# NVlabs/EmerNeRF

Hardware: NVIDIA H100
Metric: training rays/sec (8192-ray batch) (higher is better)
Workload: dtype f32

## Files before the change

### emernerf_b200/csrc/field_wgrad.cu

```cuda
#include "common.cuh"
#include "tc_common.cuh"

namespace emer {
namespace fw {

using namespace emer::tc;

constexpr int TR = 16;
constexpr int STAGES = 3;
constexpr int THREADS = 384;
constexpr int PROD_REGS = 56, CONS_REGS = 224;
constexpr int MIN_TILES = 4;

constexpr int BAR_FULL = 1, BAR_EMPTY = 3, BAR_RING = 5, BAR_PROD = 5 + STAGES;

constexpr int PANEL64 = TR * 64 * 4, PANEL8 = TR * 8 * 4;
constexpr int P_DZB = 0, P_DF = 2 * PANEL64, P_DSEM = 4 * PANEL64, P_DZ0 = 6 * PANEL64, P_DZ1 = 8 * PANEL64,
              P_DZ2 = 10 * PANEL64, P_BYTES = P_DZ2 + 2 * PANEL8;

template <int KE, bool HEAD>
struct Stage {
    static constexpr int LD_ENC = KE + 4, LD64 = 68, LD128 = 132, LD_D1 = HEAD ? LD128 : LD64;
    static constexpr int ENC = 0, HB = ENC + TR * LD_ENC, DZB = HB + TR * LD64, DSEM = DZB + TR * LD64,
                         D1 = DSEM + TR * LD64, DF = D1 + (HEAD ? 64 : 0), HG = D1 + TR * LD_D1, H1 = HG + TR * LD128,
                         DZ1 = H1 + TR * LD64, DZ2 = DZ1 + TR * LD64;
    static constexpr int FLOATS = HEAD ? DZ2 + TR * 3 : HG;
};

struct Params {
    const float* enc; int64_t ld_enc;
    const float *hb, *hg, *h1, *dz2, *dz1, *d1, *dzb, *d_sem;
    float *dwb0, *dbb0, *dwb1, *dbb1;
    float *dw0g, *dw1h, *dw1g; int64_t ld_w0, ld_w1;
    float *dw2, *db2;
    int64_t n;
};

__device__ __forceinline__ void cp_async16(float* dst, const float* src, int bytes) {
    asm volatile("cp.async.cg.shared.global [%0], [%1], 16, %2;\n" ::"r"(smem_u32(dst)), "l"(src), "r"(bytes) : "memory");
}
__device__ __forceinline__ void cp_async_commit() { asm volatile("cp.async.commit_group;\n" ::: "memory"); }
template <int N>
__device__ __forceinline__ void cp_async_wait() { asm volatile("cp.async.wait_group %0;\n" ::"n"(N) : "memory"); }
__device__ __forceinline__ void bar_sync(int id, int count) { asm volatile("bar.sync %0, %1;\n" ::"r"(id), "r"(count) : "memory"); }
__device__ __forceinline__ void bar_arrive(int id, int count) { asm volatile("bar.arrive %0, %1;\n" ::"r"(id), "r"(count) : "memory"); }

template <int W>
__device__ __forceinline__ void copy_rows(float* dst, const float* src, int64_t ld, int64_t row0, int rows_left, int t) {
    constexpr int CPR = W / 4, CHUNKS = TR * CPR;
    const float* s = src + row0 * ld;
#pragma unroll
    for (int k = 0; k < (CHUNKS + 127) / 128; ++k) {
        const int c = t + 128 * k;
        if (CHUNKS % 128 == 0 || c < CHUNKS) {
            const int r = c / CPR, j = c % CPR;
            const bool ok = r < rows_left;
            cp_async16(dst + r * (W + 4) + 4 * j, ok ? s + r * ld + 4 * j : src, ok ? 16 : 0);
        }
    }
}

template <int B, int KE, bool HEAD>
__device__ __forceinline__ void split_col(const float* st, uint8_t* pan, int col, bool sem, float& dbs) {
    using S = Stage<KE, HEAD>;
    constexpr int soff = B == 0 ? S::DZB : B == 1 ? S::DF : B == 2 ? S::DSEM : B == 3 ? S::D1 : B == 4 ? S::DZ1 : S::DZ2;
    constexpr int sld = B == 1 || B == 3 ? S::LD_D1 : (B == 5 ? 3 : S::LD64);
    constexpr int rows = B == 5 ? 8 : 64;
    constexpr int pb = B == 0 ? P_DZB : B == 1 ? P_DF : B == 2 ? P_DSEM : B == 3 ? P_DZ0 : B == 4 ? P_DZ1 : P_DZ2;
    if constexpr (B >= 3 && !HEAD) return;
    if ((B == 2 && !sem) || (B == 5 && col >= 8)) return;
    const bool real = B != 5 || col < 3;
    const float* z = st + soff + (real ? col : 0);
#pragma unroll
    for (int ks = 0; ks < 2; ++ks) {
#pragma unroll
        for (int h = 0; h < 2; ++h) {
            float v[4], hi[4], lo[4];
#pragma unroll
            for (int j = 0; j < 4; ++j) {
                v[j] = real ? z[(8 * ks + 2 * j + h) * sld] : 0.0f;
                split(v[j], hi[j], lo[j]);
                dbs += v[j];
            }
            uint8_t* dst = pan + pb + (2 * ks + h) * rows * 16 + col * 16;
            *reinterpret_cast<float4*>(dst) = make_float4(hi[0], hi[1], hi[2], hi[3]);
            *reinterpret_cast<float4*>(dst + TR * rows * 4) = make_float4(lo[0], lo[1], lo[2], lo[3]);
        }
    }
}

template <int FV>
__device__ __forceinline__ void load_a(const float* x, int ld, int f0, int q, uint32_t (&hi)[2][4], uint32_t (&lo)[2][4]) {
    const int f1 = f0 + 8;
#pragma unroll
    for (int ks = 0; ks < 2; ++ks) {
        const float* ra = x + (8 * ks + 2 * q) * ld;
        const float* rb = ra + ld;
        frag_split(f0 < FV ? ra[f0] : 0.0f, f0 < FV ? rb[f0] : 0.0f, f1 < FV ? ra[f1] : 0.0f, f1 < FV ? rb[f1] : 0.0f,
                   hi[ks], lo[ks]);
    }
}

template <int N>
__device__ __forceinline__ void mma_tile(float (&acc)[N / 2], const uint32_t (&hi)[2][4], const uint32_t (&lo)[2][4],
                                         uint32_t panel) {
#pragma unroll
    for (int ks = 0; ks < 2; ++ks)
        mma3<N>(acc, hi[ks], lo[ks], b_desc(panel, N, ks, 0), b_desc(panel + TR * N * 4, N, ks, 0), 1);
}

template <int N>
__device__ __forceinline__ void flush(const float (&acc)[N / 2], float* dw, int64_t ld, int fv, int ov, int f0, int q) {
#pragma unroll
    for (int j = 0; j < N / 8; ++j) {
#pragma unroll
        for (int e = 0; e < 4; ++e) {
            const int f = e < 2 ? f0 : f0 + 8, o = 8 * j + 2 * q + (e & 1);
            if (f < fv && o < ov) atomicAdd(dw + (int64_t)o * ld + f, acc[4 * j + e]);
        }
    }
}

template <int KE, bool HEAD>
__global__ void __launch_bounds__(THREADS, 1) field_wgrad_kernel(const __grid_constant__ Params p) {
    using S = Stage<KE, HEAD>;
    extern __shared__ __align__(128) uint8_t smem[];
    float* ring = reinterpret_cast<float*>(smem + 2 * P_BYTES);
    const int tid = threadIdx.x, lane = tid & 31, q = lane & 3;
    const int wgi = __shfl_sync(0xffffffffu, tid >> 7, 0);
    const bool sem = p.d_sem != nullptr;
    const int64_t n_tiles = (p.n + TR - 1) / TR;
    const int64_t my_tiles = (n_tiles - blockIdx.x + gridDim.x - 1) / gridDim.x;

    if (wgi == 0) {
        asm volatile("setmaxnreg.dec.sync.aligned.u32 %0;\n" ::"n"(PROD_REGS));
        auto issue = [&](int64_t i, int slot) {
            if (i < my_tiles) {
                const int64_t row0 = (blockIdx.x + i * gridDim.x) * TR;
                const int rows_left = p.n - row0 < TR ? (int)(p.n - row0) : TR;
                float* st = ring + slot * S::FLOATS;
                copy_rows<KE>(st + S::ENC, p.enc, p.ld_enc, row0, rows_left, tid);
                copy_rows<64>(st + S::HB, p.hb, 64, row0, rows_left, tid);
                copy_rows<64>(st + S::DZB, p.dzb, 64, row0, rows_left, tid);
                if (sem) copy_rows<64>(st + S::DSEM, p.d_sem, 64, row0, rows_left, tid);
                copy_rows<HEAD ? 128 : 64>(st + S::D1, p.d1 + (HEAD ? 0 : 64), 128, row0, rows_left, tid);
                if constexpr (HEAD) {
                    copy_rows<128>(st + S::HG, p.hg, 128, row0, rows_left, tid);
                    copy_rows<64>(st + S::H1, p.h1, 64, row0, rows_left, tid);
                    copy_rows<64>(st + S::DZ1, p.dz1, 64, row0, rows_left, tid);
                    if (tid < TR * 3 / 4) {
                        const int left = rows_left * 12 - 16 * tid;
                        const int b = left <= 0 ? 0 : (left < 16 ? left : 16);
                        cp_async16(st + S::DZ2 + 4 * tid, b ? p.dz2 + row0 * 3 + 4 * tid : p.dz2, b);
                    }
                }
            }
            cp_async_commit();
        };
        const int col = tid & 63, half = __shfl_sync(0xffffffffu, tid >> 6, 0);
        float db0 = 0.0f, db1 = 0.0f, db2 = 0.0f;
        issue(0, 0);
        issue(1, 1);
        int slot = 0;
        for (int64_t i = 0; i < my_tiles; ++i, slot = slot + 1 == STAGES ? 0 : slot + 1) {
            const int pb = (int)(i & 1), prev = slot == 0 ? STAGES - 1 : slot - 1;
            if (i >= 1 && i + 2 < my_tiles) bar_sync(BAR_RING + prev, THREADS);
            issue(i + 2, prev);
            if (i >= 2) bar_sync(BAR_EMPTY + pb, THREADS);
            cp_async_wait<2>();
            bar_sync(BAR_PROD, 128);
            const float* st = ring + slot * S::FLOATS;
            uint8_t* pan = smem + pb * P_BYTES;
            if (half == 0) {
                split_col<0, KE, HEAD>(st, pan, col, sem, db0);
                split_col<2, KE, HEAD>(st, pan, col, sem, db1);
                split_col<4, KE, HEAD>(st, pan, col, sem, db2);
            } else {
                split_col<1, KE, HEAD>(st, pan, col, sem, db0);
                split_col<3, KE, HEAD>(st, pan, col, sem, db1);
                split_col<5, KE, HEAD>(st, pan, col, sem, db2);
            }
            fence_async_proxy();
            bar_arrive(BAR_FULL + pb, THREADS);
        }
        cp_async_wait<0>();
        if (half == 0) {
            atomicAdd(p.dbb0 + col, db0);
            if (sem) atomicAdd(p.dbb1 + 64 + col, db1);
        } else {
            atomicAdd(p.dbb1 + col, db0);
            if (HEAD && col < 3) atomicAdd(p.db2 + col, db2);
        }
    } else {
        asm volatile("setmaxnreg.inc.sync.aligned.u32 %0;\n" ::"n"(CONS_REGS));
        const uint32_t pan0 = smem_u32(smem);
        const int f0 = 16 * ((tid >> 5) & 3) + (lane >> 2);
        float a0[32], a1[32], a2[32], a3[4];
#pragma unroll
        for (int i = 0; i < 32; ++i) a0[i] = a1[i] = a2[i] = 0.0f;
#pragma unroll
        for (int i = 0; i < 4; ++i) a3[i] = 0.0f;

        int slot = 0;
        for (int64_t i = 0; i < my_tiles; ++i, slot = slot + 1 == STAGES ? 0 : slot + 1) {
            const int pb = (int)(i & 1);
            bar_sync(BAR_FULL + pb, THREADS);
            const float* st = ring + slot * S::FLOATS;
            const uint32_t pan = pan0 + (uint32_t)pb * P_BYTES;
            uint32_t h0[2][4], l0[2][4], h1[2][4], l1[2][4], h2[2][4], l2[2][4];
            if (wgi == 1) {
                load_a<KE>(st + S::ENC, S::LD_ENC, f0, q, h0, l0);
                if (HEAD) load_a<64>(st + S::HG + 64, S::LD128, f0, q, h1, l1);
            } else {
                load_a<64>(st + S::HB, S::LD64, f0, q, h0, l0);
                if (HEAD) {
                    load_a<64>(st + S::HG, S::LD128, f0, q, h1, l1);
                    load_a<64>(st + S::H1, S::LD64, f0, q, h2, l2);
                }
            }
            if (i + STAGES < my_tiles) bar_arrive(BAR_RING + slot, THREADS);
            wg_fence();
            if (wgi == 1) {
                mma_tile<64>(a0, h0, l0, pan + P_DZB);
                if (HEAD) {
                    mma_tile<64>(a1, h1, l1, pan + P_DZ0);
                    mma_tile<64>(a2, h1, l1, pan + P_DZ1);
                }
            } else {
                mma_tile<64>(a0, h0, l0, pan + P_DF);
                if (sem) mma_tile<64>(a2, h0, l0, pan + P_DSEM);
                if (HEAD) {
                    mma_tile<64>(a1, h1, l1, pan + P_DZ1);
                    mma_tile<8>(a3, h2, l2, pan + P_DZ2);
                }
            }
            wg_commit();
            wg_wait0();
            if (i + 2 < my_tiles) bar_arrive(BAR_EMPTY + pb, THREADS);
        }

        if (wgi == 1) {
            flush<64>(a0, p.dwb0, KE, KE, 64, f0, q);
            if (HEAD) {
                flush<64>(a1, p.dw0g, p.ld_w0, 64, 64, f0, q);
                flush<64>(a2, p.dw1g, p.ld_w1, 64, 64, f0, q);
            }
        } else {
            flush<64>(a0, p.dwb1, 64, 64, 64, f0, q);
            if (sem) flush<64>(a2, p.dwb1 + 64 * 64, 64, 64, 64, f0, q);
            if (HEAD) {
                flush<64>(a1, p.dw1h, p.ld_w1, 64, 64, f0, q);
                flush<8>(a3, p.dw2, 64, 64, 3, f0, q);
            }
        }
    }
}

template <int KE, bool HEAD>
static int launch_t(const Params& p, cudaStream_t st) {
    constexpr int smem = 2 * P_BYTES + STAGES * Stage<KE, HEAD>::FLOATS * 4;
    static_assert(smem <= 227 * 1024, "field_wgrad_kernel: shared memory");
    static bool configured[64] = {false};
    const int dev = current_device();
    if (!configured[dev]) {
        cudaError_t e = cudaFuncSetAttribute(field_wgrad_kernel<KE, HEAD>, cudaFuncAttributeMaxDynamicSharedMemorySize, smem);
        if (e != cudaSuccess) {
            set_error("emer_field_wgrad: cudaFuncSetAttribute(%d): %s", smem, cudaGetErrorString(e));
            return -2;
        }
        configured[dev] = true;
    }
    int64_t grid = sm_count();
    const int64_t ctas = ceil_div(ceil_div(p.n, TR), MIN_TILES);
    if (grid > ctas) grid = ctas;
    field_wgrad_kernel<KE, HEAD><<<(unsigned)grid, THREADS, smem, st>>>(p);
    return check_launch("emer_field_wgrad");
}

template <bool HEAD>
static int launch_h(const Params& p, int k_enc, cudaStream_t st) {
    if (k_enc == 32) return launch_t<32, HEAD>(p, st);
    if (k_enc == 40) return launch_t<40, HEAD>(p, st);
    return launch_t<64, HEAD>(p, st);
}

}
}

extern "C" int emer_field_wgrad(const float* enc, int64_t ld_enc, int k_enc, const float* hb, const float* hg,
                                const float* h1, const float* dz2, const float* dz1, const float* d1, const float* dzb,
                                const float* d_sem, int n_feat, float* dwb0, float* dbb0, float* dwb1, float* dbb1,
                                float* dw0g, int64_t ld_w0, float* dw1h, float* dw1g, int64_t ld_w1, float* dw2,
                                float* db2, int64_t n, void* stream) {
    if (n == 0) return 0;
    EMER_REQUIRE(enc && hb && d1 && dzb && dwb0 && dbb0 && dwb1 && dbb1, "emer_field_wgrad: NULL pointer");
    EMER_REQUIRE(!dz2 || (hg && h1 && dz1 && dw0g && dw1h && dw1g && dw2 && db2),
                 "emer_field_wgrad: NULL pointer among the colour head's buffers");
    EMER_REQUIRE(k_enc == 32 || k_enc == 40 || k_enc == 64, "emer_field_wgrad: k_enc=%d must be 32, 40 or 64", k_enc);
    EMER_REQUIRE(n_feat == 64 || n_feat == 128, "emer_field_wgrad: n_feat=%d must be 64 or 128", n_feat);
    EMER_REQUIRE(!d_sem || n_feat == 128, "emer_field_wgrad: d_sem needs n_feat = 128");
    EMER_REQUIRE(ld_enc % 4 == 0 && ld_enc >= k_enc, "emer_field_wgrad: ld_enc=%lld (need a multiple of 4, >= k_enc)",
                 (long long)ld_enc);
    EMER_REQUIRE(!dz2 || (ld_w0 >= 64 && ld_w1 >= 64), "emer_field_wgrad: ld_w0=%lld ld_w1=%lld shorter than a block",
                 (long long)ld_w0, (long long)ld_w1);
    EMER_REQUIRE((((uintptr_t)enc | (uintptr_t)hb | (uintptr_t)hg | (uintptr_t)h1 | (uintptr_t)dz2 | (uintptr_t)dz1 |
                   (uintptr_t)d1 | (uintptr_t)dzb | (uintptr_t)d_sem) & 15) == 0,
                 "emer_field_wgrad: row buffers must be 16-byte aligned");
    emer::fw::Params p{enc, ld_enc, hb, hg, h1, dz2, dz1, d1, dzb, d_sem, dwb0, dbb0, dwb1, dbb1,
                       dw0g, dw1h, dw1g, ld_w0, ld_w1, dw2, db2, n};
    const cudaStream_t st = (cudaStream_t)stream;
    return dz2 ? emer::fw::launch_h<true>(p, k_enc, st) : emer::fw::launch_h<false>(p, k_enc, st);
}
```

Measured before the change: 2.287 million.

## Load weight-gradient row tiles with TMA and mbarriers, double-buffer consumer fragments

Replaces the per-thread cp.async row copies in the producer warpgroup with TMA bulk tensor copies issued by a single thread and tracked by per-slot mbarriers with expected transaction bytes. Consumers now also wait on the mbarrier. The consumer loop is restructured to load the next tile's A fragments while the current wgmma runs. This aims to cut producer instruction overhead and overlap fragment loads with the MMAs, at the cost of host-side tensor-map encoding on every launch, more consumer registers, and an int32 row limit.

```diff
diff --git a/emernerf_b200/csrc/field_wgrad.cu b/emernerf_b200/csrc/field_wgrad.cu
--- a/emernerf_b200/csrc/field_wgrad.cu
+++ b/emernerf_b200/csrc/field_wgrad.cu
@@ -1,3 +1,6 @@
+#include <cuda.h>
+#include <cudaTypedefs.h>
+
 #include "common.cuh"
 #include "tc_common.cuh"
 
@@ -12,7 +15,7 @@
 constexpr int PROD_REGS = 56, CONS_REGS = 224;
 constexpr int MIN_TILES = 4;
 
-constexpr int BAR_FULL = 1, BAR_EMPTY = 3, BAR_RING = 5, BAR_PROD = 5 + STAGES;
+constexpr int BAR_FULL = 1, BAR_EMPTY = 3, BAR_RING = 5, RING_COUNT = 256 + 32;
 
 constexpr int PANEL64 = TR * 64 * 4, PANEL8 = TR * 8 * 4;
 constexpr int P_DZB = 0, P_DF = 2 * PANEL64, P_DSEM = 4 * PANEL64, P_DZ0 = 6 * PANEL64, P_DZ1 = 8 * PANEL64,
@@ -24,40 +27,42 @@
     static constexpr int ENC = 0, HB = ENC + TR * LD_ENC, DZB = HB + TR * LD64, DSEM = DZB + TR * LD64,
                          D1 = DSEM + TR * LD64, DF = D1 + (HEAD ? 64 : 0), HG = D1 + TR * LD_D1, H1 = HG + TR * LD128,
                          DZ1 = H1 + TR * LD64, DZ2 = DZ1 + TR * LD64;
-    static constexpr int FLOATS = HEAD ? DZ2 + TR * 3 : HG;
+    static constexpr int FLOATS = HEAD ? DZ2 + 64 : HG;
+    static constexpr int TX_BYTES = 4 * TR * (LD_ENC + 2 * LD64 + LD_D1 + (HEAD ? LD128 + 2 * LD64 : 0)) + (HEAD ? 4 * TR * 3 : 0);
+    static constexpr int TX_SEM = 4 * TR * LD64;
 };
 
 struct Params {
-    const float* enc; int64_t ld_enc;
-    const float *hb, *hg, *h1, *dz2, *dz1, *d1, *dzb, *d_sem;
+    CUtensorMap enc, hb, dzb, d_sem, d1, hg, h1, dz1, dz2;
+    bool sem;
     float *dwb0, *dbb0, *dwb1, *dbb1;
     float *dw0g, *dw1h, *dw1g; int64_t ld_w0, ld_w1;
     float *dw2, *db2;
     int64_t n;
 };
 
-__device__ __forceinline__ void cp_async16(float* dst, const float* src, int bytes) {
-    asm volatile("cp.async.cg.shared.global [%0], [%1], 16, %2;\n" ::"r"(smem_u32(dst)), "l"(src), "r"(bytes) : "memory");
-}
-__device__ __forceinline__ void cp_async_commit() { asm volatile("cp.async.commit_group;\n" ::: "memory"); }
-template <int N>
-__device__ __forceinline__ void cp_async_wait() { asm volatile("cp.async.wait_group %0;\n" ::"n"(N) : "memory"); }
 __device__ __forceinline__ void bar_sync(int id, int count) { asm volatile("bar.sync %0, %1;\n" ::"r"(id), "r"(count) : "memory"); }
 __device__ __forceinline__ void bar_arrive(int id, int count) { asm volatile("bar.arrive %0, %1;\n" ::"r"(id), "r"(count) : "memory"); }
 
-template <int W>
-__device__ __forceinline__ void copy_rows(float* dst, const float* src, int64_t ld, int64_t row0, int rows_left, int t) {
-    constexpr int CPR = W / 4, CHUNKS = TR * CPR;
-    const float* s = src + row0 * ld;
-#pragma unroll
-    for (int k = 0; k < (CHUNKS + 127) / 128; ++k) {
-        const int c = t + 128 * k;
-        if (CHUNKS % 128 == 0 || c < CHUNKS) {
-            const int r = c / CPR, j = c % CPR;
-            const bool ok = r < rows_left;
-            cp_async16(dst + r * (W + 4) + 4 * j, ok ? s + r * ld + 4 * j : src, ok ? 16 : 0);
-        }
-    }
+__device__ __forceinline__ void mbar_init(uint32_t bar, int count) {
+    asm volatile("mbarrier.init.shared::cta.b64 [%0], %1;\n" ::"r"(bar), "r"(count) : "memory");
+}
+__device__ __forceinline__ void mbar_arrive_tx(uint32_t bar, int bytes) {
+    asm volatile("mbarrier.arrive.expect_tx.shared::cta.b64 _, [%0], %1;\n" ::"r"(bar), "r"(bytes) : "memory");
+}
+__device__ __forceinline__ void mbar_wait(uint32_t bar, uint32_t parity) {
+    asm volatile(
+        "{\n.reg .pred p;\nWAIT:\n"
+        "mbarrier.try_wait.parity.shared::cta.b64 p, [%0], %1;\n"
+        "@!p bra WAIT;\n}\n" ::"r"(bar), "r"(parity) : "memory");
+}
+__device__ __forceinline__ void copy_box(float* dst, const CUtensorMap& m, int row0, uint32_t bar) {
+    asm volatile("cp.async.bulk.tensor.2d.shared::cluster.global.mbarrier::complete_tx::bytes [%0], [%1, {%2, %3}], [%4];\n"
+                 ::"r"(smem_u32(dst)), "l"(&m), "r"(0), "r"(row0), "r"(bar) : "memory");
+}
+__device__ __forceinline__ void copy_box_1d(float* dst, const CUtensorMap& m, int x0, uint32_t bar) {
+    asm volatile("cp.async.bulk.tensor.1d.shared::cluster.global.mbarrier::complete_tx::bytes [%0], [%1, {%2}], [%3];\n"
+                 ::"r"(smem_u32(dst)), "l"(&m), "r"(x0), "r"(bar) : "memory");
 }
 
 template <int B, int KE, bool HEAD>
@@ -126,49 +131,55 @@
     using S = Stage<KE, HEAD>;
     extern __shared__ __align__(128) uint8_t smem[];
     float* ring = reinterpret_cast<float*>(smem + 2 * P_BYTES);
+    const uint32_t landed = smem_u32(ring + STAGES * S::FLOATS);
     const int tid = threadIdx.x, lane = tid & 31, q = lane & 3;
     const int wgi = __shfl_sync(0xffffffffu, tid >> 7, 0);
-    const bool sem = p.d_sem != nullptr;
+    const bool sem = p.sem;
     const int64_t n_tiles = (p.n + TR - 1) / TR;
     const int64_t my_tiles = (n_tiles - blockIdx.x + gridDim.x - 1) / gridDim.x;
+
+    if (tid < STAGES) mbar_init(landed + 8 * tid, 1);
+    asm volatile("fence.mbarrier_init.release.cluster;\n" ::: "memory");
+    __syncthreads();
 
     if (wgi == 0) {
         asm volatile("setmaxnreg.dec.sync.aligned.u32 %0;\n" ::"n"(PROD_REGS));
         auto issue = [&](int64_t i, int slot) {
-            if (i < my_tiles) {
-                const int64_t row0 = (blockIdx.x + i * gridDim.x) * TR;
-                const int rows_left = p.n - row0 < TR ? (int)(p.n - row0) : TR;
-                float* st = ring + slot * S::FLOATS;
-                copy_rows<KE>(st + S::ENC, p.enc, p.ld_enc, row0, rows_left, tid);
-                copy_rows<64>(st + S::HB, p.hb, 64, row0, rows_left, tid);
-                copy_rows<64>(st + S::DZB, p.dzb, 64, row0, rows_left, tid);
-                if (sem) copy_rows<64>(st + S::DSEM, p.d_sem, 64, row0, rows_left, tid);
-                copy_rows<HEAD ? 128 : 64>(st + S::D1, p.d1 + (HEAD ? 0 : 64), 128, row0, rows_left, tid);
-                if constexpr (HEAD) {
-                    copy_rows<128>(st + S::HG, p.hg, 128, row0, rows_left, tid);
-                    copy_rows<64>(st + S::H1, p.h1, 64, row0, rows_left, tid);
-                    copy_rows<64>(st + S::DZ1, p.dz1, 64, row0, rows_left, tid);
-                    if (tid < TR * 3 / 4) {
-                        const int left = rows_left * 12 - 16 * tid;
-                        const int b = left <= 0 ? 0 : (left < 16 ? left : 16);
-                        cp_async16(st + S::DZ2 + 4 * tid, b ? p.dz2 + row0 * 3 + 4 * tid : p.dz2, b);
-                    }
-                }
-            }
-            cp_async_commit();
+            const int row0 = (int)((blockIdx.x + i * gridDim.x) * TR);
+            const uint32_t bar = landed + 8 * slot;
+            float* st = ring + slot * S::FLOATS;
+            fence_async_proxy();
+            mbar_arrive_tx(bar, S::TX_BYTES + (sem ? S::TX_SEM : 0));
+            copy_box(st + S::ENC, p.enc, row0, bar);
+            copy_box(st + S::HB, p.hb, row0, bar);
+            copy_box(st + S::DZB, p.dzb, row0, bar);
+            if (sem) copy_box(st + S::DSEM, p.d_sem, row0, bar);
+            copy_box(st + S::D1, p.d1, row0, bar);
+            if constexpr (HEAD) {
+                copy_box(st + S::HG, p.hg, row0, bar);
+                copy_box(st + S::H1, p.h1, row0, bar);
+                copy_box(st + S::DZ1, p.dz1, row0, bar);
+                copy_box_1d(st + S::DZ2, p.dz2, row0 * 3, bar);
+            }
         };
         const int col = tid & 63, half = __shfl_sync(0xffffffffu, tid >> 6, 0);
+        const bool issuer = __shfl_sync(0xffffffffu, tid < 32, 0);
         float db0 = 0.0f, db1 = 0.0f, db2 = 0.0f;
-        issue(0, 0);
-        issue(1, 1);
+        if (tid == 0) {
+            if (my_tiles > 0) issue(0, 0);
+            if (my_tiles > 1) issue(1, 1);
+        }
         int slot = 0;
-        for (int64_t i = 0; i < my_tiles; ++i, slot = slot + 1 == STAGES ? 0 : slot + 1) {
+        uint32_t phase = 0;
+        for (int64_t i = 0; i < my_tiles; ++i) {
             const int pb = (int)(i & 1), prev = slot == 0 ? STAGES - 1 : slot - 1;
-            if (i >= 1 && i + 2 < my_tiles) bar_sync(BAR_RING + prev, THREADS);
-            issue(i + 2, prev);
+            if (issuer && i + 2 < my_tiles) {
+                if (i >= 1) bar_sync(BAR_RING + prev, RING_COUNT);
+                if (lane == 0) issue(i + 2, prev);
+                __syncwarp();
+            }
+            mbar_wait(landed + 8 * slot, phase);
             if (i >= 2) bar_sync(BAR_EMPTY + pb, THREADS);
-            cp_async_wait<2>();
-            bar_sync(BAR_PROD, 128);
             const float* st = ring + slot * S::FLOATS;
             uint8_t* pan = smem + pb * P_BYTES;
             if (half == 0) {
@@ -182,8 +193,8 @@
             }
             fence_async_proxy();
             bar_arrive(BAR_FULL + pb, THREADS);
-        }
-        cp_async_wait<0>();
+            if (++slot == STAGES) slot = 0, phase ^= 1;
+        }
         if (half == 0) {
             atomicAdd(p.dbb0 + col, db0);
             if (sem) atomicAdd(p.dbb1 + 64 + col, db1);
@@ -201,42 +212,56 @@
 #pragma unroll
         for (int i = 0; i < 4; ++i) a3[i] = 0.0f;
 
+        struct Frags { uint32_t h0[2][4], l0[2][4], h1[2][4], l1[2][4], h2[2][4], l2[2][4]; };
         int slot = 0;
-        for (int64_t i = 0; i < my_tiles; ++i, slot = slot + 1 == STAGES ? 0 : slot + 1) {
-            const int pb = (int)(i & 1);
-            bar_sync(BAR_FULL + pb, THREADS);
+        uint32_t phase = 0;
+        auto load = [&](int64_t i, Frags& a) {
+            bar_sync(BAR_FULL + (int)(i & 1), THREADS);
+            mbar_wait(landed + 8 * slot, phase);
             const float* st = ring + slot * S::FLOATS;
-            const uint32_t pan = pan0 + (uint32_t)pb * P_BYTES;
-            uint32_t h0[2][4], l0[2][4], h1[2][4], l1[2][4], h2[2][4], l2[2][4];
             if (wgi == 1) {
-                load_a<KE>(st + S::ENC, S::LD_ENC, f0, q, h0, l0);
-                if (HEAD) load_a<64>(st + S::HG + 64, S::LD128, f0, q, h1, l1);
+                load_a<KE>(st + S::ENC, S::LD_ENC, f0, q, a.h0, a.l0);
+                if (HEAD) load_a<64>(st + S::HG + 64, S::LD128, f0, q, a.h1, a.l1);
             } else {
-                load_a<64>(st + S::HB, S::LD64, f0, q, h0, l0);
+                load_a<64>(st + S::HB, S::LD64, f0, q, a.h0, a.l0);
                 if (HEAD) {
-                    load_a<64>(st + S::HG, S::LD128, f0, q, h1, l1);
-                    load_a<64>(st + S::H1, S::LD64, f0, q, h2, l2);
+                    load_a<64>(st + S::HG, S::LD128, f0, q, a.h1, a.l1);
+                    load_a<64>(st + S::H1, S::LD64, f0, q, a.h2, a.l2);
                 }
             }
-            if (i + STAGES < my_tiles) bar_arrive(BAR_RING + slot, THREADS);
+            if (i + STAGES < my_tiles) bar_arrive(BAR_RING + slot, RING_COUNT);
+            if (++slot == STAGES) slot = 0, phase ^= 1;
+        };
+        auto mma = [&](int64_t i, const Frags& a) {
+            const uint32_t pan = pan0 + (uint32_t)(i & 1) * P_BYTES;
             wg_fence();
             if (wgi == 1) {
-                mma_tile<64>(a0, h0, l0, pan + P_DZB);
+                mma_tile<64>(a0, a.h0, a.l0, pan + P_DZB);
                 if (HEAD) {
-                    mma_tile<64>(a1, h1, l1, pan + P_DZ0);
-                    mma_tile<64>(a2, h1, l1, pan + P_DZ1);
+                    mma_tile<64>(a1, a.h1, a.l1, pan + P_DZ0);
+                    mma_tile<64>(a2, a.h1, a.l1, pan + P_DZ1);
                 }
             } else {
-                mma_tile<64>(a0, h0, l0, pan + P_DF);
-                if (sem) mma_tile<64>(a2, h0, l0, pan + P_DSEM);
+                mma_tile<64>(a0, a.h0, a.l0, pan + P_DF);
+                if (sem) mma_tile<64>(a2, a.h0, a.l0, pan + P_DSEM);
                 if (HEAD) {
-                    mma_tile<64>(a1, h1, l1, pan + P_DZ1);
-                    mma_tile<8>(a3, h2, l2, pan + P_DZ2);
+                    mma_tile<64>(a1, a.h1, a.l1, pan + P_DZ1);
+                    mma_tile<8>(a3, a.h2, a.l2, pan + P_DZ2);
                 }
             }
             wg_commit();
+        };
+        auto step = [&](int64_t i, const Frags& cur, Frags& nxt) {
+            mma(i, cur);
+            if (i + 1 < my_tiles) load(i + 1, nxt);
             wg_wait0();
-            if (i + 2 < my_tiles) bar_arrive(BAR_EMPTY + pb, THREADS);
+            if (i + 2 < my_tiles) bar_arrive(BAR_EMPTY + (int)(i & 1), THREADS);
+        };
+        Frags fa, fb;
+        if (my_tiles > 0) load(0, fa);
+        for (int64_t i = 0; i < my_tiles; i += 2) {
+            step(i, fa, fb);
+            if (i + 1 < my_tiles) step(i + 1, fb, fa);
         }
 
         if (wgi == 1) {
@@ -256,10 +281,58 @@
     }
 }
 
+struct Rows {
+    const float* enc; int64_t ld_enc;
+    const float *hb, *hg, *h1, *dz2, *dz1, *d1, *dzb, *d_sem;
+};
+
+using EncodeTiled = PFN_cuTensorMapEncodeTiled_v12000;
+static EncodeTiled encoder() {
+    static const EncodeTiled fn = [] {
+        void* f = nullptr;
+        cudaDriverEntryPointQueryResult q;
+        if (cudaGetDriverEntryPointByVersion("cuTensorMapEncodeTiled", &f, 12000, cudaEnableDefault, &q) != cudaSuccess ||
+            q != cudaDriverEntryPointSuccess)
+            f = nullptr;
+        return (EncodeTiled)f;
+    }();
+    return fn;
+}
+static bool tensor_map(EncodeTiled encode, CUtensorMap* m, const float* base, int rank, int64_t cols, int64_t n,
+                       int64_t ld, int box) {
+    const cuuint64_t dim[2] = {(cuuint64_t)cols, (cuuint64_t)n}, stride[1] = {(cuuint64_t)ld * 4};
+    const cuuint32_t boxd[2] = {(cuuint32_t)box, (cuuint32_t)TR}, elem[2] = {1, 1};
+    return encode(m, CU_TENSOR_MAP_DATA_TYPE_FLOAT32, (cuuint32_t)rank, const_cast<float*>(base), dim, stride, boxd, elem,
+                  CU_TENSOR_MAP_INTERLEAVE_NONE, CU_TENSOR_MAP_SWIZZLE_NONE, CU_TENSOR_MAP_L2_PROMOTION_L2_256B,
+                  CU_TENSOR_MAP_FLOAT_OOB_FILL_NONE) == CUDA_SUCCESS;
+}
+
 template <int KE, bool HEAD>
-static int launch_t(const Params& p, cudaStream_t st) {
-    constexpr int smem = 2 * P_BYTES + STAGES * Stage<KE, HEAD>::FLOATS * 4;
+static int launch_t(Params p, const Rows& r, cudaStream_t st) {
+    using S = Stage<KE, HEAD>;
+    constexpr int smem = 2 * P_BYTES + STAGES * S::FLOATS * 4 + STAGES * 8;
     static_assert(smem <= 227 * 1024, "field_wgrad_kernel: shared memory");
+    static_assert((2 * P_BYTES) % 128 == 0 && (S::FLOATS * 4) % 128 == 0, "field_wgrad_kernel: ring slots 128-byte aligned");
+    const EncodeTiled encode = encoder();
+    if (!encode) {
+        set_error("emer_field_wgrad: cuTensorMapEncodeTiled is not available from the driver");
+        return -2;
+    }
+    const int64_t n = p.n;
+    bool ok = tensor_map(encode, &p.enc, r.enc, 2, KE, n, r.ld_enc, S::LD_ENC) &&
+              tensor_map(encode, &p.hb, r.hb, 2, 64, n, 64, S::LD64) &&
+              tensor_map(encode, &p.dzb, r.dzb, 2, 64, n, 64, S::LD64) &&
+              (!p.sem || tensor_map(encode, &p.d_sem, r.d_sem, 2, 64, n, 64, S::LD64)) &&
+              tensor_map(encode, &p.d1, HEAD ? r.d1 : r.d1 + 64, 2, HEAD ? 128 : 64, n, 128, S::LD_D1);
+    if (HEAD)
+        ok = ok && tensor_map(encode, &p.hg, r.hg, 2, 128, n, 128, S::LD128) &&
+             tensor_map(encode, &p.h1, r.h1, 2, 64, n, 64, S::LD64) &&
+             tensor_map(encode, &p.dz1, r.dz1, 2, 64, n, 64, S::LD64) &&
+             tensor_map(encode, &p.dz2, r.dz2, 1, 3 * n, 1, 1, TR * 3);
+    if (!ok) {
+        set_error("emer_field_wgrad: cuTensorMapEncodeTiled failed (n=%lld)", (long long)n);
+        return -2;
+    }
     static bool configured[64] = {false};
     const int dev = current_device();
     if (!configured[dev]) {
@@ -278,10 +351,10 @@
 }
 
 template <bool HEAD>
-static int launch_h(const Params& p, int k_enc, cudaStream_t st) {
-    if (k_enc == 32) return launch_t<32, HEAD>(p, st);
-    if (k_enc == 40) return launch_t<40, HEAD>(p, st);
-    return launch_t<64, HEAD>(p, st);
+static int launch_h(const Params& p, const Rows& r, int k_enc, cudaStream_t st) {
+    if (k_enc == 32) return launch_t<32, HEAD>(p, r, st);
+    if (k_enc == 40) return launch_t<40, HEAD>(p, r, st);
+    return launch_t<64, HEAD>(p, r, st);
 }
 
 }
@@ -306,8 +379,12 @@
     EMER_REQUIRE((((uintptr_t)enc | (uintptr_t)hb | (uintptr_t)hg | (uintptr_t)h1 | (uintptr_t)dz2 | (uintptr_t)dz1 |
                    (uintptr_t)d1 | (uintptr_t)dzb | (uintptr_t)d_sem) & 15) == 0,
                  "emer_field_wgrad: row buffers must be 16-byte aligned");
-    emer::fw::Params p{enc, ld_enc, hb, hg, h1, dz2, dz1, d1, dzb, d_sem, dwb0, dbb0, dwb1, dbb1,
-                       dw0g, dw1h, dw1g, ld_w0, ld_w1, dw2, db2, n};
+    EMER_REQUIRE(n <= INT32_MAX / 3, "emer_field_wgrad: n=%lld rows (at most 2^31 / 3)", (long long)n);
+    emer::fw::Params p{};
+    p.sem = d_sem != nullptr;
+    p.dwb0 = dwb0, p.dbb0 = dbb0, p.dwb1 = dwb1, p.dbb1 = dbb1;
+    p.dw0g = dw0g, p.dw1h = dw1h, p.dw1g = dw1g, p.ld_w0 = ld_w0, p.ld_w1 = ld_w1, p.dw2 = dw2, p.db2 = db2, p.n = n;
+    const emer::fw::Rows r{enc, ld_enc, hb, hg, h1, dz2, dz1, d1, dzb, d_sem};
     const cudaStream_t st = (cudaStream_t)stream;
-    return dz2 ? emer::fw::launch_h<true>(p, k_enc, st) : emer::fw::launch_h<false>(p, k_enc, st);
-}
+    return dz2 ? emer::fw::launch_h<true>(p, r, k_enc, st) : emer::fw::launch_h<false>(p, r, k_enc, st);
+}
```

Result: faster. 2.362 million, median of 6 (+3.3%).
